# dazzmo/ik

Measured on AMD Instinct MI355X. Metric: IK solves/sec (50-iter DLS) at batch=65536, higher is better.
Workload: dtype f64; 1 GPU; Cassie single-leg chain (cassie_fixed.urdf, 7 support joints of nq=16), one SE(3) LeftFootFront task, 50 fixed DLS iterations, damping 1e-2, step 1.0, reachable targets FK(q*); batch_per_gpu=65536, global_batch=65536, kernel=dls_chain<NJ=7,full,hot>, parallelism=single GPU

## Files before the change

### ik_amd/csrc/device/chain_hot.hpp

```cpp
#pragma once
#if !defined(__HIPCC_RTC__)
#include <cstdint>
#endif

#include "chain_kernel_body.hpp"

namespace ikdev {

constexpr int kStructBits = 21;
constexpr int kStructPerWord = 3;
enum : unsigned { kEntGeneral = 0, kEntZero = 1, kEntOne = 2, kEntMinusOne = 3 };

template <uint64_t C0, uint64_t C1, uint64_t C2>
struct ChainStruct {
    static constexpr uint64_t word(int w) { return w == 0 ? C0 : (w == 1 ? C1 : C2); }
    static constexpr unsigned code(int i) { return static_cast<unsigned>((word(i / kStructPerWord) >> (kStructBits * (i % kStructPerWord))) & 0x1fffffu); }
    static constexpr unsigned ent(int i, int e) { return (code(i) >> (2 * e)) & 3u; }
    static constexpr bool tnz(int i, int k) { return ((code(i) >> (18 + k)) & 1u) != 0; }
    static constexpr int ngen_before(int i, int e) { return e == 0 ? 0 : ngen_before(i, e - 1) + (ent(i, e - 1) == kEntGeneral ? 1 : 0); }
    static constexpr int count(int i) { return ngen_before(i, 9) + (tnz(i, 0) ? 1 : 0) + (tnz(i, 1) ? 1 : 0) + (tnz(i, 2) ? 1 : 0); }
    static constexpr int offset(int i) { return i == 0 ? 0 : offset(i - 1) + count(i - 1); }
    static constexpr int rot_at(int i, int e) { return offset(i) + ngen_before(i, e); }
    static constexpr int trans_at(int i, int k) {
        return offset(i) + ngen_before(i, 9) + (k > 0 && tnz(i, 0) ? 1 : 0) + (k > 1 && tnz(i, 1) ? 1 : 0);
// ... 93 lines not shown
                if (S::tnz(jj, 0)) {                                                                       \
                    const double t0 = t.v[S::trans_at(jj, 0)];                                             \
                    p[0] = dfma(cs[jj], t0, p[0]); p[1] = dfma(-sn[jj], t0, p[1]);                         \
                }                                                                                          \
                if (S::tnz(jj, 1)) {                                                                       \
                    const double t1 = t.v[S::trans_at(jj, 1)];                                             \
                    p[0] = dfma(sn[jj], t1, p[0]); p[1] = dfma(cs[jj], t1, p[1]);                          \
                }                                                                                          \
                if (S::tnz(jj, 2)) p[2] += t.v[S::trans_at(jj, 2)];                                        \
            } else {                                                                                       \
                                       \
                _Pragma("unroll") for (int k = 0; k < 6; ++k) rows[jj][k] = R[k];                          \
                rot_z_left(R, p, sn[jj], cs[jj]);                                                          \
                hot_compose_left<S, jj>(R, p, t);                                                          \
                if (kPinWalk) { IKD_PIN(p[0]); IKD_PIN(p[1]); IKD_PIN(p[2]); IKD_PIN(R[0]); }              \
            }                                                                                              \
        }                                                                                                  \
    }
    IKD_HOT_JOINT(6) IKD_HOT_JOINT(5) IKD_HOT_JOINT(4) IKD_HOT_JOINT(3) IKD_HOT_JOINT(2) IKD_HOT_JOINT(1) IKD_HOT_JOINT(0)
#undef IKD_HOT_JOINT

    if (kRuns.any_folded) { IKD_PIN(p[0]); IKD_PIN(p[1]); }
    double Re[9], pe[3];
#pragma unroll
    for (int i = 0; i < 3; ++i)
#pragma unroll
        for (int j = 0; j < 3; ++j) Re[3 * i + j] = dfma(R[i], oMt[j], dfma(R[3 + i], oMt[3 + j], R[6 + i] * oMt[6 + j]));
    {
        const double dp[3] = {oMt[9] - p[0], oMt[10] - p[1], oMt[11] - p[2]};
        rotT_vec(R, dp, pe);
    }
    LogAndJlog lj;
    double Cm[9];
    log6_and_jlog6_hot<false>(Re, pe, lj, &Cm);
#pragma unroll
    for (int i = 0; i < 6; ++i) e[i] = lj.e[i];

    double Ar0[NJ][3], Ar1[NJ][3];
#pragma unroll
    for (int j = 0; j < NJ; ++j)
        if (kRuns.folded[j] && kRuns.leader[j] == j) {
#pragma unroll
            for (int i = 0; i < 3; ++i) {
                Ar0[j][i] = dfma(lj.A[3 * i], rows[j][0], dfma(lj.A[3 * i + 1], rows[j][1], lj.A[3 * i + 2] * rows[j][2]));
                Ar1[j][i] = dfma(lj.A[3 * i], rows[j][3], dfma(lj.A[3 * i + 1], rows[j][4], lj.A[3 * i + 2] * rows[j][5]));
            }
        }

#pragma unroll
    for (int j = 0; j < NJ; ++j) {
        double beta[3];
#pragma unroll
        for (int i = 0; i < 3; ++i) beta[i] = dfma(lj.A[3 * i], ang[j][0], dfma(lj.A[3 * i + 1], ang[j][1], lj.A[3 * i + 2] * ang[j][2]));
#pragma unroll
        for (int i = 0; i < 3; ++i) {
            const double cb = dfma(Cm[3 * i], beta[0], dfma(Cm[3 * i + 1], beta[1], Cm[3 * i + 2] * beta[2]));
            if (!kRuns.folded[j])
            col[j][i] = dfma(lj.A[3 * i], lin[j][0], dfma(lj.A[3 * i + 1], lin[j][1], dfma(lj.A[3 * i + 2], lin[j][2], cb)));
            else
                col[j][i] = dfma(pt[j][0], Ar1[kRuns.leader[j]][i], dfma(-pt[j][1], Ar0[kRuns.leader[j]][i], cb));
            col[j][3 + i] = beta[i];
        }
    }
}

template <int NJ, class S>
IKD_FN void hot_gram(const double (&col)[NJ][6], double lam2, double (&G)[36]) {
// ... 47 lines not shown
IKD_FN void hot_step(const Tab &t, const LoopParams &prm, const double (&col)[NJ][6], const double (&y)[6], double (&q)[NJ], bool take) {
    constexpr int kLim = S::offset(NJ + 1);
    constexpr typename ChainRuns<S, NJ>::Table kRuns = ChainRuns<S, NJ>::value;
    double ang[NJ];
#pragma unroll
    for (int j = 0; j < NJ; ++j)
        if (kRuns.leader[j] == j) ang[j] = dfma(col[j][3], y[3], dfma(col[j][4], y[4], col[j][5] * y[5]));
#pragma unroll
    for (int j = 0; j < NJ; ++j) {
        double s = ang[kRuns.leader[j]];
#pragma unroll
        for (int a = 0; a < 3; ++a) s = dfma(col[j][a], y[a], s);
        const double qn = dfma(prm.step_length, s, q[j]);
        const double qc = dmin(t.v[kLim + NJ + j], dmax(qn, t.v[kLim + j]));
        q[j] = take ? qc : q[j];
    }
}

template <int NJ, class S, bool NEVERSTOP, class Tab, class AnyFn>
IKD_FN void hot_dls(const Tab &t, const LoopParams &prm, double (&q)[NJ], const double (&oMt)[12], int &iters_out,
                    bool &success_out, AnyFn any_active) {
    constexpr int M = 6;
    bool active = true;
    bool success = false;
    int iters = prm.max_iterations;
#pragma unroll 1
    for (int it = 0; it < prm.max_iterations; ++it) {
        double e[M], col[NJ][M];
        hot_evaluate<NJ, S>(t, q, oMt, e, col);

        double G[M * M];
        hot_gram<NJ, S>(col, prm.lam2, G);
        double y[M];
        chol_solve<M>(G, e, y);

        if (!NEVERSTOP) {
            double e0sq = 0.0;
            if (prm.priority == 0) {
#pragma unroll
                for (int a = 0; a < M; ++a) e0sq = dfma(e[a], e[a], e0sq);
            }
            const bool stop_now = active && (prm.stop_sq_tol >= 0.0) && (e0sq < prm.stop_sq_tol);
            if (stop_now) { success = true; iters = it; }
            active = active && !stop_now;
        }
        hot_step<NJ, S>(t, prm, col, y, q, NEVERSTOP || active);
        if (!NEVERSTOP && !any_active(active)) break;
    }
    iters_out = (NEVERSTOP || success) ? iters : iterations_taken(any_active, prm.max_iterations);
    success_out = success;
}

template <int NJ>
IKD_FN void hot_pass_through_from(const ChainKernelArgs<NJ> &a, const double *q_src, double *q_out, int64_t b, bool stepped) {
    constexpr int kGroup = 16;
    for (int i0 = 0; i0 < a.nq; i0 += kGroup) {
        double v[kGroup], lo[kGroup], hi[kGroup];
        bool out[kGroup];
#pragma unroll
        for (int k = 0; k < kGroup; ++k) {
            const int i = i0 + k < a.nq ? i0 + k : a.nq - 1;
            out[k] = i0 + k < a.nq && !a.q_in_chain[i];
            v[k] = q_src[at(a.layout, a.B, a.nq, i, b)];
            lo[k] = a.lower[i];
            hi[k] = a.upper[i];
        }
#pragma unroll
        for (int k = 0; k < kGroup; ++k) {
            const double c = dmin(hi[k], dmax(v[k], lo[k]));
            if (out[k]) q_out[at(a.layout, a.B, a.nq, i0 + k, b)] = stepped ? c : v[k];
        }
    }
}
template <int NJ>
IKD_FN void hot_pass_through_to(const ChainKernelArgs<NJ> &a, double *q_out, int64_t b, bool stepped) { hot_pass_through_from(a, a.q0, q_out, b, stepped); }
template <int NJ>
IKD_FN void hot_pass_through(const ChainKernelArgs<NJ> &a, int64_t b, bool stepped) { hot_pass_through_to(a, a.q_out, b, stepped); }

#if IKD_HIP_LANG
template <int NJ, class S, class Tab>
__device__ __forceinline__ void hot_refill_body(const ChainKernelArgs<NJ> &a, const Tab &t, unsigned long long *queue, int chunk) {
    chain_refill_loop<NJ>(a, queue, chunk, [&](double (&q)[NJ], const double (&oMt)[12], bool have) {
        constexpr int M = 6;
        double e[M], col[NJ][M];
        hot_evaluate<NJ, S>(t, q, oMt, e, col);
        double G[M * M];
        hot_gram<NJ, S>(col, a.prm.lam2, G);
        double y[M];
        chol_solve<M>(G, e, y);
        double e0sq = 0.0;
        if (a.prm.priority == 0) {
#pragma unroll
            for (int k = 0; k < M; ++k) e0sq = dfma(e[k], e[k], e0sq);
        }
        const bool stop_now = have && (a.prm.stop_sq_tol >= 0.0) && (e0sq < a.prm.stop_sq_tol);
        hot_step<NJ, S>(t, a.prm, col, y, q, !stop_now);
        return stop_now;
    });
}
#endif

template <int NJ, class S, bool NEVERSTOP, class Tab, class AnyFn>
IKD_FN void hot_chain_body(const ChainKernelArgs<NJ> &a, const Tab &t, int64_t gid, AnyFn any_active) {
#if defined(IKGPU_HOT_STAMP) && IKD_ON_DEVICE
    const long long rs = wall_clock64();
#endif
    const bool valid = gid < a.B;
    const int64_t b = valid ? gid : a.B - 1;
    double q[NJ];
#pragma unroll
    for (int j = 0; j < NJ; ++j) q[j] = a.q0[at(a.layout, a.B, a.nq, a.qidx[j], b)];
    double oMt[12];
    load_target(a, b, oMt);
    if (NEVERSTOP && valid) hot_pass_through(a, b, a.prm.max_iterations > 0);
    int iters;
    bool success;
#if defined(IKGPU_HOT_STAMP) && IKD_ON_DEVICE
    const long long c0 = __builtin_readcyclecounter(), r0 = wall_clock64();
#endif
    hot_dls<NJ, S, NEVERSTOP>(t, a.prm, q, oMt, iters, success, any_active);
#if defined(IKGPU_HOT_STAMP) && IKD_ON_DEVICE
    const long long c1 = __builtin_readcyclecounter(), r1 = wall_clock64();
    const int stamp_loop_cycles = static_cast<int>(c1 - c0), stamp_loop_ticks = static_cast<int>(r1 - r0);
    const int stamp_pre_ticks = static_cast<int>(r0 - rs);
    const int stamp_true_iters = iters;
#endif
    if (!NEVERSTOP && a.append_count)
        append_unfinished(a.append_list, a.append_count, valid && !success && iters < a.prm.max_iterations, b);
    if (!valid) return;
#pragma unroll
    for (int j = 0; j < NJ; ++j) a.q_out[at(a.layout, a.B, a.nq, a.qidx[j], b)] = q[j];
    if (!NEVERSTOP) hot_pass_through(a, b, iters > 0);
    if (a.success) a.success[b] = success ? 1 : 0;
#if defined(IKGPU_HOT_STAMP) && IKD_ON_DEVICE
    {
        asm volatile("s_waitcnt vmcnt(0)" ::: "memory");
        const long long re = wall_clock64();
        const int lane = threadIdx.x % 64;
        iters = lane == 0 ? stamp_loop_cycles : lane == 1 ? stamp_loop_ticks : lane == 2 ? stamp_pre_ticks
              : lane == 3 ? static_cast<int>(re - r1) : lane == 4 ? static_cast<int>(rs & 0x7fffffff)
              : lane == 5 ? static_cast<int>(re & 0x7fffffff) : stamp_true_iters;
    }
#endif
    if (a.iters) a.iters[b] = iters;
}

template <int NJ, class S, bool NEVERSTOP, class Tab, class AnyFn>
IKD_FN void hot_track_body(const ChainKernelArgs<NJ> &a, const Tab &t, int T, int64_t gid, AnyFn any_active) {
    const bool valid = gid < a.B;
    const int64_t b = valid ? gid : a.B - 1;
    const int64_t q_slab = static_cast<int64_t>(a.nq) * a.B, t_slab = 12 * a.B;
    double q[NJ];
#pragma unroll
    for (int j = 0; j < NJ; ++j) q[j] = a.q0[at(a.layout, a.B, a.nq, a.qidx[j], b)];
    double next[12], oMt[12];
    if (T > 0) {
        load_target_raw(a, a.targets, b, next);
        compose_target(a, next, oMt);
    }
    if (T > 1) load_target_raw(a, a.targets + t_slab, b, next);
    bool stepped = NEVERSTOP && a.prm.max_iterations > 0;
    for (int k = 0; k < T; ++k) {
        double *q_out = a.q_out + k * q_slab;
        if (NEVERSTOP && valid) hot_pass_through_to(a, q_out, b, stepped);
        int iters;
        bool success;
        hot_dls<NJ, S, NEVERSTOP>(t, a.prm, q, oMt, iters, success, any_active);
        stepped = stepped || iters > 0;
        if (k + 1 < T) compose_target(a, next, oMt);
        if (valid) {
#pragma unroll
            for (int j = 0; j < NJ; ++j) q_out[at(a.layout, a.B, a.nq, a.qidx[j], b)] = q[j];
            if (a.success) a.success[k * a.B + b] = success ? 1 : 0;
            if (a.iters) a.iters[k * a.B + b] = iters;
            if (!NEVERSTOP) hot_pass_through_to(a, q_out, b, stepped);
        }
        if (k + 2 < T) load_target_raw(a, a.targets + (k + 2) * t_slab, b, next);
    }
}

template <int NJ, class S, bool NEVERSTOP, class Tab, class AnyFn>
IKD_FN void hot_multistart_lane(const ChainKernelArgs<NJ> &a, const MultistartArgs &ms, const Tab &t, int64_t b, int k, double (&q)[NJ],
                                bool &success, int &iters, double &err_sq, AnyFn any_active) {
    multistart_load(a, ms, b, k, q);
    double oMt[12];
    load_target(a, b, oMt);
    hot_dls<NJ, S, NEVERSTOP>(t, a.prm, q, oMt, iters, success, any_active);
    double e[6], col[NJ][6];
    hot_evaluate<NJ, S>(t, q, oMt, e, col);
    err_sq = 0.0;
#pragma unroll
    for (int r = 0; r < 6; ++r) err_sq = dfma(e[r], e[r], err_sq);
}

template <int NJ, class S, bool NEVERSTOP, class Tab, class AnyFn, class Exchange>
IKD_FN void hot_multistart_body(const ChainKernelArgs<NJ> &a, const MultistartArgs &ms, const Tab &t, int64_t gid, AnyFn any_active,
                                Exchange exchange) {
    const int64_t prob = gid >> ms.log2K;
    const int k = static_cast<int>(gid & ((int64_t{1} << ms.log2K) - 1));
    const bool valid = prob < a.B;
    const int64_t b = valid ? prob : a.B - 1;
    double q[NJ], err_sq;
    bool success;
    int iters;
    hot_multistart_lane<NJ, S, NEVERSTOP>(a, ms, t, b, k, q, success, iters, err_sq, any_active);
// ... 94 lines not shown
```

### ik_amd/csrc/device/chain_kernel_body.hpp

```cpp
#pragma once
#if !defined(__HIPCC_RTC__)
#include <cstdint>
#endif

#include "chain_solver.hpp"
#include "multistart.hpp"
#include "solutions.hpp"

namespace ikdev {

enum : int { LAYOUT_SOA = 0, LAYOUT_AOS = 1 };

template <int NJ>
struct ChainKernelArgs {
    const ChainDesc<NJ> *desc;
    LoopParams prm;
    double ref_pl[12];
    int qidx[NJ];
    int vidx[NJ];
    int nq, nv, layout;
    int64_t B;
    const double *q0;
    const double *targets;
    double *q_out;
    uint8_t *success;
    int32_t *iters;
    const double *lower, *upper;
    const uint8_t *q_in_chain;
    double *e_out, *J_out, *oMf_out;
    const int32_t *worklist;
    const unsigned long long *count;
    int leave_active, leave_after;
    int32_t *append_list;
    unsigned long long *append_count;
};

IKD_FN void append_unfinished(int32_t *list, unsigned long long *count, bool open, int64_t b) {
#if IKD_ON_DEVICE
    const unsigned long long mask = __ballot(open);
    if (mask == 0ull) return;
    const int lane = static_cast<int>(threadIdx.x) & 63;
    unsigned long long base = 0;
    if (lane == __ffsll(static_cast<long long>(mask)) - 1) base = atomicAdd(count, static_cast<unsigned long long>(__popcll(mask)));
    const int src = __ffsll(static_cast<long long>(mask)) - 1;
    const unsigned lo = __shfl(static_cast<unsigned>(base), src), hi = __shfl(static_cast<unsigned>(base >> 32), src);
    base = (static_cast<unsigned long long>(hi) << 32) | lo;
    if (open) list[base + __popcll(mask & ((1ull << lane) - 1ull))] = static_cast<int32_t>(b);
#else
    if (open) list[(*count)++] = static_cast<int32_t>(b);
#endif
}

IKD_FN int64_t at(int layout, int64_t B, int ncomp, int c, int64_t b) {
    return layout == LAYOUT_SOA ? static_cast<int64_t>(c) * B + b : b * ncomp + c;
}

template <int NJ>
IKD_FN void load_target(const ChainKernelArgs<NJ> &a, int64_t b, double (&oMt)[12]) {
    double t[12];
#pragma unroll
    for (int k = 0; k < 12; ++k) t[k] = a.targets[at(a.layout, a.B, 12, k, b)];
    const double *r = a.ref_pl;
#pragma unroll
    for (int i = 0; i < 3; ++i) {
#pragma unroll
        for (int j = 0; j < 3; ++j)
            oMt[3 * i + j] = dfma(r[3 * i], t[j], dfma(r[3 * i + 1], t[3 + j], r[3 * i + 2] * t[6 + j]));
        oMt[9 + i] = dfma(r[3 * i], t[9], dfma(r[3 * i + 1], t[10], dfma(r[3 * i + 2], t[11], r[9 + i])));
    }
}

template <int NJ, int KT, int SMASK = -1, class Desc, class AnyFn>
IKD_FN void dls_chain_body(const ChainKernelArgs<NJ> &a, const Desc &d, int64_t gid, AnyFn any_active) {
    const bool valid = gid < a.B;
    const int64_t b = valid ? gid : a.B - 1;

    double q[NJ];
#pragma unroll
    for (int j = 0; j < NJ; ++j) q[j] = a.q0[at(a.layout, a.B, a.nq, a.qidx[j], b)];
    double oMt[12];
    load_target(a, b, oMt);

    int iters;
    bool success;
    chain_dls<NJ, KT, SMASK>(d, a.prm, q, oMt, iters, success, any_active);

    if (a.append_count) append_unfinished(a.append_list, a.append_count, valid && !success && iters < a.prm.max_iterations, b);
    if (!valid) return;
#pragma unroll
    for (int j = 0; j < NJ; ++j) a.q_out[at(a.layout, a.B, a.nq, a.qidx[j], b)] = q[j];
    for (int i = 0; i < a.nq; ++i) {
        if (a.q_in_chain[i]) continue;
        const double v = a.q0[at(a.layout, a.B, a.nq, i, b)];
        const double c = dmin(a.upper[i], dmax(v, a.lower[i]));
        a.q_out[at(a.layout, a.B, a.nq, i, b)] = (iters > 0) ? c : v;
    }
    if (a.success) a.success[b] = success ? 1 : 0;
    if (a.iters) a.iters[b] = iters;
}

template <int NJ>
IKD_FN void load_target_raw(const ChainKernelArgs<NJ> &a, const double *targets, int64_t b, double (&t)[12]) {
#pragma unroll
    for (int k = 0; k < 12; ++k) t[k] = targets[at(a.layout, a.B, 12, k, b)];
}
template <int NJ>
IKD_FN void compose_target(const ChainKernelArgs<NJ> &a, const double (&t)[12], double (&oMt)[12]) {
    const double *r = a.ref_pl;
#pragma unroll
    for (int i = 0; i < 3; ++i) {
#pragma unroll
        for (int j = 0; j < 3; ++j)
            oMt[3 * i + j] = dfma(r[3 * i], t[j], dfma(r[3 * i + 1], t[3 + j], r[3 * i + 2] * t[6 + j]));
        oMt[9 + i] = dfma(r[3 * i], t[9], dfma(r[3 * i + 1], t[10], dfma(r[3 * i + 2], t[11], r[9 + i])));
    }
}

template <int NJ, int KT, int SMASK = -1, class Desc, class AnyFn>
IKD_FN void dls_chain_track_body(const ChainKernelArgs<NJ> &a, const Desc &d, int T, int64_t gid, AnyFn any_active) {
    const bool valid = gid < a.B;
    const int64_t b = valid ? gid : a.B - 1;
    const int64_t q_slab = static_cast<int64_t>(a.nq) * a.B, t_slab = 12 * a.B;

    double q[NJ];
#pragma unroll
    for (int j = 0; j < NJ; ++j) q[j] = a.q0[at(a.layout, a.B, a.nq, a.qidx[j], b)];
    double next[12], oMt[12];
    if (T > 0) {
        load_target_raw(a, a.targets, b, next);
        compose_target(a, next, oMt);
    }
    if (T > 1) load_target_raw(a, a.targets + t_slab, b, next);
    bool stepped = false;
    for (int k = 0; k < T; ++k) {
        int iters;
        bool success;
        chain_dls<NJ, KT, SMASK>(d, a.prm, q, oMt, iters, success, any_active);
        stepped = stepped || iters > 0;
        if (k + 1 < T) compose_target(a, next, oMt);
        if (valid) {
            double *q_out = a.q_out + k * q_slab;
#pragma unroll
            for (int j = 0; j < NJ; ++j) q_out[at(a.layout, a.B, a.nq, a.qidx[j], b)] = q[j];
            if (a.success) a.success[k * a.B + b] = success ? 1 : 0;
            if (a.iters) a.iters[k * a.B + b] = iters;
            for (int i = 0; i < a.nq; ++i) {
                if (a.q_in_chain[i]) continue;
                const double v = a.q0[at(a.layout, a.B, a.nq, i, b)];
                const double c = dmin(a.upper[i], dmax(v, a.lower[i]));
                q_out[at(a.layout, a.B, a.nq, i, b)] = stepped ? c : v;
            }
        }
        if (k + 2 < T) load_target_raw(a, a.targets + (k + 2) * t_slab, b, next);
    }
}


template <int NJ>
IKD_FN const double *multistart_source(const ChainKernelArgs<NJ> &a, const MultistartArgs &ms, int k) {
    return (k == 0 || !ms.starts) ? a.q0 : ms.starts + static_cast<int64_t>(k - 1) * a.nq * a.B;
}

template <int NJ>
IKD_FN void multistart_load(const ChainKernelArgs<NJ> &a, const MultistartArgs &ms, int64_t b, int k, double (&q)[NJ]) {
    const double *src = multistart_source(a, ms, k);
    const bool generated = k > 0 && !ms.starts;
#pragma unroll
    for (int j = 0; j < NJ; ++j) {
        const int i = a.qidx[j];
        const double v = src[at(a.layout, a.B, a.nq, i, b)];
        const double r = multistart_draw(ms.seed, b, k, i, a.lower[i], a.upper[i]);
        q[j] = (generated && ms.draw[i]) ? r : v;
    }
}

template <int NJ, int KT, int SMASK = -1, class Desc, class AnyFn>
IKD_FN void dls_chain_multistart_lane(const ChainKernelArgs<NJ> &a, const MultistartArgs &ms, const Desc &d, int64_t b, int k,
                                      double (&q)[NJ], bool &success, int &iters, double &err_sq, AnyFn any_active) {
    constexpr int M = TaskDim<KT>::value;
    multistart_load(a, ms, b, k, q);
    double oMt[12];
    load_target(a, b, oMt);
    chain_dls<NJ, KT, SMASK>(d, a.prm, q, oMt, iters, success, any_active);
    double e[M], col[NJ][M], Rf[9], pf[3];
    chain_evaluate<NJ, KT, SMASK>(d, q, oMt, a.prm.idmask, a.prm.unit_weights != 0, e, col, Rf, pf);
    err_sq = 0.0;
#pragma unroll
    for (int r = 0; r < M; ++r) err_sq = dfma(e[r], e[r], err_sq);
}

template <int NJ, class Pass>
IKD_FN void multistart_store(const ChainKernelArgs<NJ> &a, const MultistartArgs &ms, int64_t b, int k, const double (&q)[NJ], bool success,
                             int iters, double err_sq, Pass pass) {
#pragma unroll
    for (int j = 0; j < NJ; ++j) a.q_out[at(a.layout, a.B, a.nq, a.qidx[j], b)] = q[j];
    pass(multistart_source(a, ms, k), iters > 0);
    if (a.success) a.success[b] = success ? 1 : 0;
    if (a.iters) a.iters[b] = iters;
    if (ms.winner) ms.winner[b] = k;
    if (ms.err_sq) ms.err_sq[b] = err_sq;
}

template <int NJ>
IKD_FN void chain_pass_through_from(const ChainKernelArgs<NJ> &a, const double *src, int64_t b, bool stepped) {
    for (int i = 0; i < a.nq; ++i) {
        if (a.q_in_chain[i]) continue;
        const double v = src[at(a.layout, a.B, a.nq, i, b)];
        const double c = dmin(a.upper[i], dmax(v, a.lower[i]));
        a.q_out[at(a.layout, a.B, a.nq, i, b)] = stepped ? c : v;
    }
}

template <int NJ, int KT, int SMASK = -1, class Desc, class AnyFn, class Exchange>
IKD_FN void dls_chain_multistart_body(const ChainKernelArgs<NJ> &a, const MultistartArgs &ms, const Desc &d, int64_t gid, AnyFn any_active,
                                      Exchange exchange) {
    const int64_t prob = gid >> ms.log2K;
    const int k = static_cast<int>(gid & ((int64_t{1} << ms.log2K) - 1));
    const bool valid = prob < a.B;
    const int64_t b = valid ? prob : a.B - 1;
    double q[NJ], err_sq;
    bool success;
    int iters;
    dls_chain_multistart_lane<NJ, KT, SMASK>(a, ms, d, b, k, q, success, iters, err_sq, any_active);
    const int win = multistart_select(ms.log2K, multistart_key(success, err_sq), k, exchange);
    if (valid && win == k)
        multistart_store(a, ms, b, k, q, success, iters, err_sq, [&](const double *src, bool stepped) { chain_pass_through_from(a, src, b, stepped); });
}


template <int NJ>
IKD_FN void chain_pass_through_into(const ChainKernelArgs<NJ> &a, const double *src, double *q_out, int64_t b, bool stepped) {
    for (int i = 0; i < a.nq; ++i) {
        if (a.q_in_chain[i]) continue;
        const double v = src[at(a.layout, a.B, a.nq, i, b)];
        const double c = dmin(a.upper[i], dmax(v, a.lower[i]));
        q_out[at(a.layout, a.B, a.nq, i, b)] = stepped ? c : v;
    }
}

template <int NJ, int KT, int SMASK = -1, class Desc, class AnyFn>
IKD_FN void dls_chain_solutions_lane(const ChainKernelArgs<NJ> &a, const SolutionsArgs &sa, const Desc &d, int64_t b, int k, double (&q)[NJ],
                                     bool &success, int &iters, AnyFn any_active) {
    multistart_load(a, sa.ms, b, k, q);
    double oMt[12];
    load_target(a, b, oMt);
    chain_dls<NJ, KT, SMASK>(d, a.prm, q, oMt, iters, success, any_active);
}

template <int NJ, class Pass>
IKD_FN void solutions_store(const ChainKernelArgs<NJ> &a, const SolutionsArgs &sa, int64_t b, int k, int slot, const double (&q)[NJ], int iters,
                            Pass pass) {
    double *q_out = a.q_out + static_cast<int64_t>(slot) * a.nq * a.B;
    pass(multistart_source(a, sa.ms, k), q_out, iters > 0);
#pragma unroll
    for (int j = 0; j < NJ; ++j) q_out[at(a.layout, a.B, a.nq, a.qidx[j], b)] = q[j];
    if (sa.which) sa.which[slot * a.B + b] = k;
    if (a.iters) a.iters[slot * a.B + b] = iters;
}

template <int NJ, int KT, int SMASK = -1, class Desc, class AnyFn, class Fetch>
IKD_FN void dls_chain_solutions_body(const ChainKernelArgs<NJ> &a, const SolutionsArgs &sa, const Desc &d, int64_t gid, AnyFn any_active,
                                     Fetch fetch) {
    const int64_t prob = gid >> sa.ms.log2K;
    const int k = static_cast<int>(gid & ((int64_t{1} << sa.ms.log2K) - 1));
    const bool valid = prob < a.B;
    const int64_t b = valid ? prob : a.B - 1;
    double q[NJ];
    bool success;
    int iters;
    dls_chain_solutions_lane<NJ, KT, SMASK>(a, sa, d, b, k, q, success, iters, any_active);
    SolutionsLane s;
    solutions_select<NJ>(s, sa.ms.log2K, k, sa.N, sa.sep, success, q, fetch);
    if (!valid) return;
    if (s.kept)
        solutions_store(a, sa, b, k, s.slot, q, iters,
                        [&](const double *src, double *q_out, bool stepped) { chain_pass_through_into(a, src, q_out, b, stepped); });
    if (k == 0) sa.count[b] = s.cnt;
}

#if IKD_HIP_LANG
template <int NJ, class IterFn>
__device__ __forceinline__ void chain_refill_loop(const ChainKernelArgs<NJ> &a, unsigned long long *queue, int chunk_and_batch, IterFn iterate) {
    const int lane = static_cast<int>(threadIdx.x) & 63;
    const int64_t first_round = static_cast<int64_t>(gridDim.x) * 64;
    const bool listed = a.worklist != nullptr;
    const int64_t nwork = listed ? static_cast<int64_t>(*a.count) : a.B;
    const double *qsrc = listed ? a.q_out : a.q0;
    auto problem = [&](int64_t w) { return listed ? static_cast<int64_t>(a.worklist[w]) : w; };
    const int64_t w0 = static_cast<int64_t>(blockIdx.x) * 64 + lane;
    bool have = w0 < nwork;
    double q[NJ], oMt[12];
    int64_t b = 0;
    int it = 0;
    const int max_it = a.prm.max_iterations;
    const int64_t working = (nwork + 63) / 64 < static_cast<int64_t>(gridDim.x) ? (nwork + 63) / 64 : static_cast<int64_t>(gridDim.x);
    if (static_cast<int64_t>(blockIdx.x) >= working) return;
    b = problem(have ? w0 : 0);
#pragma unroll
    for (int j = 0; j < NJ; ++j) q[j] = qsrc[at(a.layout, a.B, a.nq, a.qidx[j], b)];
    load_target(a, b, oMt);
    if (listed) it = a.iters[b];
    int64_t pool_lo = 0, pool_hi = 0;
    bool exhausted = first_round >= nwork;
    const int batch = chunk_and_batch >> 16, chunk = chunk_and_batch & 0xffff;
    while (__any(have)) {
        const bool stop_now = iterate(q, oMt, have) && have;
        ++it;
        const bool done = have && (stop_now || it >= max_it);
        if (done) {
#pragma unroll
            for (int j = 0; j < NJ; ++j) a.q_out[at(a.layout, a.B, a.nq, a.qidx[j], b)] = q[j];
            if (a.success) a.success[b] = stop_now ? 1 : 0;
            a.iters[b] = stop_now ? it - 1 : max_it;
            have = false;
        }
        const unsigned long long mask = __ballot(!have);
        const int need = __popcll(mask);
        const bool supply = pool_hi > pool_lo || !exhausted;
        if (supply && (need >= batch || need == 64)) {
            const int rank = __popcll(mask & ((1ull << lane) - 1ull));
            const int64_t avail = pool_hi - pool_lo;
            int64_t nb = pool_lo + rank;
            bool got = rank < avail;
            if (avail < need && !exhausted) {
                unsigned long long v = 0;
                if (lane == 0) v = atomicAdd(queue, static_cast<unsigned long long>(chunk));
                const unsigned lo = __builtin_amdgcn_readfirstlane(static_cast<unsigned>(v)), hi = __builtin_amdgcn_readfirstlane(static_cast<unsigned>(v >> 32));
                const int64_t nlo = first_round + static_cast<int64_t>((static_cast<unsigned long long>(hi) << 32) | lo);
                const int64_t nhi = nlo + chunk < nwork ? nlo + chunk : nwork;
                exhausted = nlo + chunk >= nwork;
                if (rank >= avail) { nb = nlo + (rank - avail); got = nb < nhi; }
                pool_lo = nlo + (need - avail);
                pool_hi = nhi > pool_lo ? nhi : pool_lo;
            } else {
                pool_lo += need < avail ? need : avail;
            }
            if (!have && got) {
                have = true;
                b = problem(nb);
#pragma unroll
                for (int j = 0; j < NJ; ++j) q[j] = qsrc[at(a.layout, a.B, a.nq, a.qidx[j], b)];
                load_target(a, b, oMt);
                it = listed ? a.iters[b] : 0;
            }
        }
    }
    if (lane == 0) {
        __threadfence();
        if (atomicAdd(queue + 1, 1ull) == static_cast<unsigned long long>(working) - 1ull) {
            queue[0] = 0ull;
            queue[1] = 0ull;
            queue[2] = 0ull;
            __threadfence();
        }
    }
}

template <int NJ, int KT, int SMASK, class Desc>
__device__ __forceinline__ void dls_chain_refill_body(const ChainKernelArgs<NJ> &a, const Desc &d_in, unsigned long long *queue, int chunk) {
    const Desc *dp = &d_in;
    chain_refill_loop<NJ>(a, queue, chunk, [&](double (&q)[NJ], const double (&oMt)[12], bool) {
        asm volatile("" ::: "memory");
        if constexpr (!std::is_same<Desc, ChainDesc<NJ>>::value) IKD_LAUNDER(dp);
        return chain_iteration<NJ, KT, SMASK>(*dp, a.prm, q, oMt, true);
    });
}

#endif

template <int NJ, int KT>
IKD_FN void eval_chain_body(const ChainKernelArgs<NJ> &a, const ChainDesc<NJ> &d, int64_t b) {
    constexpr int M = TaskDim<KT>::value;
    if (b >= a.B) return;
    double q[NJ];
// ... 42 lines not shown
```

### ik_amd/csrc/device/chain_solver.hpp

```cpp
#pragma once
#if !defined(__HIPCC_RTC__)
#include <type_traits>
#endif

#include "lane_math.hpp"

namespace ikdev {

enum : int { KT_POSITION = 0, KT_ORIENTATION = 1, KT_FULL = 2 };

template <int NJ>
struct ChainDesc {
    double pl[NJ][12];
    double frame_pl[12];
    double lo[NJ], hi[NJ];
    double wgt[6];
};

struct LoopParams {
    int max_iterations;
    double lam2;
    double step_length;
    double stop_sq_tol;
    int priority;
// ... 119 lines not shown
        if (KT == KT_FULL || KT == KT_POSITION) {
#pragma unroll
            for (int i = 0; i < 3; ++i)
                col[j][i] = dfma(AtR[3 * i], vw[0], dfma(AtR[3 * i + 1], vw[1], dfma(AtR[3 * i + 2], vw[2],
                            dfma(BtR[3 * i], zax[j][0], dfma(BtR[3 * i + 1], zax[j][1], BtR[3 * i + 2] * zax[j][2])))));
        }
        if (KT == KT_FULL || KT == KT_ORIENTATION) {
            constexpr int r0 = (KT == KT_FULL) ? 3 : 0;
#pragma unroll
            for (int i = 0; i < 3; ++i)
                col[j][r0 + i] = dfma(AbR[3 * i], zax[j][0], dfma(AbR[3 * i + 1], zax[j][1], AbR[3 * i + 2] * zax[j][2]));
        }
    }
    (void)M;
}

template <int NJ, int KT, int SMASK = -1, class Desc>
IKD_FN bool chain_iteration(const Desc &d, const LoopParams &prm, double (&q)[NJ], const double (&oMt)[12], bool active) {
    constexpr int M = TaskDim<KT>::value;
    double e[M], col[NJ][M], Rf[9], pf[3];
    chain_evaluate<NJ, KT, SMASK>(d, q, oMt, prm.idmask, prm.unit_weights != 0, e, col, Rf, pf);

    double G[M * M];
#pragma unroll
    for (int a = 0; a < M; ++a)
#pragma unroll
        for (int b = 0; b <= a; ++b) {
            double s = (a == b) ? prm.lam2 : 0.0;
#pragma unroll
            for (int j = 0; j < NJ; ++j) s = dfma(col[j][a], col[j][b], s);
            G[a * M + b] = s;
        }
    double y[M];
    chol_solve<M>(G, e, y);

    double e0sq = 0.0;
    if (prm.priority == 0) {
#pragma unroll
        for (int a = 0; a < M; ++a) e0sq = dfma(e[a], e[a], e0sq);
    }
    const bool stop_now = active && (prm.stop_sq_tol >= 0.0) && (e0sq < prm.stop_sq_tol);
    const bool step = active && !stop_now;
#pragma unroll
    for (int j = 0; j < NJ; ++j) {
        double s = 0.0;
#pragma unroll
        for (int a = 0; a < M; ++a) s = dfma(col[j][a], y[a], s);
        const double qn = dfma(prm.step_length, s, q[j]);
        const double qc = dmin(d.hi[j], dmax(qn, d.lo[j]));
        q[j] = step ? qc : q[j];
    }
    return stop_now;
}

struct KeepGoing {
    int leave_active, leave_after, n;
    IKD_FN bool operator()(bool act) {
        ++n;
#if IKD_ON_DEVICE
        const int live = static_cast<int>(__popcll(__ballot(act)));
        return live > (n >= leave_after ? leave_active : 0);
#else
        return act;
#endif
    }
};
template <class F>
// ... 26 lines not shown
```

### ik_amd/csrc/device/lane_math.hpp

```cpp
#pragma once

#if defined(__HIPCC_RTC__)
typedef signed long long int64_t;
typedef unsigned long long uint64_t;
typedef signed int int32_t;
typedef unsigned int uint32_t;
typedef unsigned char uint8_t;
namespace std {
template <class A, class B> struct is_same { static constexpr bool value = false; };
template <class A> struct is_same<A, A> { static constexpr bool value = true; };
template <bool C, class A, class B> struct conditional { typedef A type; };
template <class A, class B> struct conditional<false, A, B> { typedef B type; };
}
#else
#include <cmath>
#include <cstdint>
#endif

#if defined(__HIPCC_RTC__)
#define IKD_FN __host__ __device__ inline __attribute__((always_inline))
#elif defined(__HIPCC__)
#include <hip/hip_runtime.h>
#define IKD_FN __host__ __device__ inline __attribute__((always_inline))
#else
// ... 330 lines not shown
    const double diag = dsel(small, 0.5 * (2.0 - t2 * (1.0 / 6.0)), 0.5 * (theta * st_omc));
#pragma unroll
    for (int i = 0; i < 3; ++i)
#pragma unroll
        for (int j = 0; j < 3; ++j) o.A[3 * i + j] = a3 * u[i] * u[j];
    o.A[0] += diag; o.A[4] += diag; o.A[8] += diag;
    o.A[1] -= 0.5 * u[2]; o.A[2] += 0.5 * u[1];
    o.A[3] += 0.5 * u[2]; o.A[5] -= 0.5 * u[0];
    o.A[6] -= 0.5 * u[1]; o.A[7] += 0.5 * u[0];

    const double inv_t2 = inv_t * inv_t;
    const double bdot = dsel(small, 1.0 / 360.0,
                             dfma(-2.0 * inv_t2, inv_t2, (1.0 + st * inv_t) * inv_t2 * (0.5 * inv_omc)));
    const double up = dot(u, pp);
    const double k1 = bdot * up, k2 = dfma(t2, bdot, 2.0 * beta);
    const double v3[3] = {dfma(k1, u[0], -(k2 * pp[0])), dfma(k1, u[1], -(k2 * pp[1])), dfma(k1, u[2], -(k2 * pp[2]))};
    double C[9];
#pragma unroll
    for (int i = 0; i < 3; ++i)
#pragma unroll
        for (int j = 0; j < 3; ++j) C[3 * i + j] = dfma(v3[i], u[j], beta * u[i] * pp[j]);
    const double ub = up * beta;
    C[0] += ub; C[4] += ub; C[8] += ub;
    C[1] -= 0.5 * pp[2]; C[2] += 0.5 * pp[1];
    C[3] += 0.5 * pp[2]; C[5] -= 0.5 * pp[0];
    C[6] -= 0.5 * pp[1]; C[7] += 0.5 * pp[0];
#pragma unroll
    for (int i = 0; i < 3; ++i)
#pragma unroll
        for (int j = 0; j < 3; ++j)
            o.Bm[3 * i + j] = dfma(C[3 * i], o.A[j], dfma(C[3 * i + 1], o.A[3 + j], C[3 * i + 2] * o.A[6 + j]));
}

template <bool WITH_BM = true>
IKD_FN void log6_and_jlog6_hot(const double (&Re)[9], const double (&pe)[3], LogAndJlog &o, double (*Cout)[9] = nullptr) {
    constexpr double pio2_hi = 1.57079632679489655800e+00, pio2_lo = 6.12323399573676603587e-17;
    constexpr double pS0 = 1.66666666666666657415e-01, pS1 = -3.25565818622400915405e-01,
                     pS2 = 2.01212532134862925881e-01, pS3 = -4.00555345006794114027e-02,
                     pS4 = 7.91534994289814532176e-04, pS5 = 3.47933107596021167570e-05;
    constexpr double qS1 = -2.40339491173441421878e+00, qS2 = 2.02094576023350569471e+00,
                     qS3 = -6.88283971605453293030e-01, qS4 = 7.70381505559019352791e-02;
    const double tr = Re[0] + Re[4] + Re[8];
    double x = dfma(tr, 0.5, -0.5);
    x = dmin(1.0, dmax(-1.0, x));
    const double ax = __builtin_fabs(x);
    const bool mid = ax < 0.5;
    const double z = dfma(-0.5, x, 0.5);
    const double zc = dmax(dfma(0.5, x, 0.5), 0x1p-104);
    const double za = mid ? x * x : dfma(-0.5, ax, 0.5);
    double pp_ = dfma3(za, pS5, pS4);
    pp_ = dfma3(za, pp_, pS3);
    pp_ = dfma3(za, pp_, pS2);
    pp_ = dfma3(za, pp_, pS1);
    pp_ = dfma3(za, pp_, pS0);
    pp_ = pp_ * za;
    double qq = dfma3(za, qS4, qS3);
    qq = dfma3(za, qq, qS2);
    qq = dfma3(za, qq, qS1);
    qq = dfma(za, qq, 1.0);
    const double rr = pp_ * drcp(qq);
    const double sa = dsqrt(za);
    const double tl = dfma(sa, rr, sa);
    const double res_mid = pio2_hi - (x - dfma(-x, rr, pio2_lo));
    const bool pos = x > 0.0;
    const double res_out = dfma(pos ? 2.0 : -2.0, tl, pos ? 0.0 : kPi);
    const double theta = mid ? res_mid : res_out;
    const double h = dsqrt(z * zc);
    const double r = drcp(dmax(theta * h, 1e-300));
    const double inv_t = r * h, inv_h = r * theta;
    const double cot = zc * inv_h;
    const bool small = theta < kTaylorPrec3;
    const double t2 = theta * theta;
    const double inv_t2 = inv_t * inv_t;

    const double fac = dsel(theta > kTaylorPrec3, 0.25 * (theta * inv_h), 0.5);
    double w[3] = {fac * (Re[7] - Re[5]), fac * (Re[2] - Re[6]), fac * (Re[3] - Re[1])};
    const bool near_pi = theta >= kPi - 1e-2;
    if (__builtin_expect(IKD_ANY(near_pi), 0)) {
        const double cphi = -x;
        const double beta_pi = t2 * drcp(2.0 * z);
        const double t0 = (Re[0] + cphi) * beta_pi, t1 = (Re[4] + cphi) * beta_pi, t2v = (Re[8] + cphi) * beta_pi;
        const double a0 = dsel(Re[7] > Re[5], 1.0, -1.0) * dsel(t0 > 0.0, dsqrt(dmax(t0, 0.0)), 0.0);
        const double a1 = dsel(Re[2] > Re[6], 1.0, -1.0) * dsel(t1 > 0.0, dsqrt(dmax(t1, 0.0)), 0.0);
        const double a2 = dsel(Re[3] > Re[1], 1.0, -1.0) * dsel(t2v > 0.0, dsqrt(dmax(t2v, 0.0)), 0.0);
        w[0] = dsel(near_pi, a0, w[0]);
        w[1] = dsel(near_pi, a1, w[1]);
        w[2] = dsel(near_pi, a2, w[2]);
    }

    const double alpha = dsel(small, 1.0 - t2 * (1.0 / 12.0) - t2 * t2 * (1.0 / 720.0), 0.5 * (theta * cot));
    const double beta = dsel(small, 1.0 / 12.0 + t2 * (1.0 / 720.0), dfma(-0.5 * inv_t, cot, inv_t2));
    double wxp[3];
    cross(w, pe, wxp);
    const double bwp = beta * dot(w, pe);
#pragma unroll
    for (int i = 0; i < 3; ++i) {
        o.e[i] = dfma(alpha, pe[i], dfma(-0.5, wxp[i], bwp * w[i]));
        o.e[3 + i] = w[i];
    }

    const double u[3] = {-w[0], -w[1], -w[2]};
    double pp[3];
    rotT_vec(Re, pe, pp);
    pp[0] = -pp[0]; pp[1] = -pp[1]; pp[2] = -pp[2];
    const double a3 = beta;
    const double diag = dsel(small, 0.5 * (2.0 - t2 * (1.0 / 6.0)), 0.5 * (theta * cot));
#pragma unroll
    for (int i = 0; i < 3; ++i)
#pragma unroll
        for (int j = 0; j < 3; ++j) o.A[3 * i + j] = a3 * u[i] * u[j];
    o.A[0] += diag; o.A[4] += diag; o.A[8] += diag;
    o.A[1] -= 0.5 * u[2]; o.A[2] += 0.5 * u[1];
    o.A[3] += 0.5 * u[2]; o.A[5] -= 0.5 * u[0];
    o.A[6] -= 0.5 * u[1]; o.A[7] += 0.5 * u[0];

    const double bdot = dsel(small, 1.0 / 360.0,
                             dfma(-2.0 * inv_t2, inv_t2, dfma(2.0 * h, inv_t, 1.0) * inv_t2 * (0.25 * (cot * inv_h))));
    const double up = dot(u, pp);
    const double k1 = bdot * up, k2 = dfma(t2, bdot, 2.0 * beta);
    const double v3[3] = {dfma(k1, u[0], -(k2 * pp[0])), dfma(k1, u[1], -(k2 * pp[1])), dfma(k1, u[2], -(k2 * pp[2]))};
    double C[9];
#pragma unroll
    for (int i = 0; i < 3; ++i)
#pragma unroll
        for (int j = 0; j < 3; ++j) C[3 * i + j] = dfma(v3[i], u[j], beta * u[i] * pp[j]);
    const double ub = up * beta;
    C[0] += ub; C[4] += ub; C[8] += ub;
    C[1] -= 0.5 * pp[2]; C[2] += 0.5 * pp[1];
    C[3] += 0.5 * pp[2]; C[5] -= 0.5 * pp[0];
    C[6] -= 0.5 * pp[1]; C[7] += 0.5 * pp[0];
    if (WITH_BM) {
#pragma unroll
        for (int i = 0; i < 3; ++i)
#pragma unroll
            for (int j = 0; j < 3; ++j)
                o.Bm[3 * i + j] = dfma(C[3 * i], o.A[j], dfma(C[3 * i + 1], o.A[3 + j], C[3 * i + 2] * o.A[6 + j]));
    } else {
#pragma unroll
        for (int k = 0; k < 9; ++k) (*Cout)[k] = C[k];
    }
}

template <int M>
IKD_FN void chol_solve(double (&G)[M * M], const double (&b)[M], double (&x)[M]) {
    double y[M];
#pragma unroll
    for (int k = 0; k < M; ++k) y[k] = b[k];
#pragma unroll
    for (int k = 0; k < M; ++k) {
        const double inv = drsqrt(G[k * M + k]);
        G[k * M + k] = inv;
        y[k] = y[k] * inv;
#pragma unroll
        for (int i = k + 1; i < M; ++i) G[i * M + k] = G[i * M + k] * inv;
#pragma unroll
        for (int i = k + 1; i < M; ++i) {
#pragma unroll
            for (int j = k + 1; j <= i; ++j) G[i * M + j] = dfma(-G[i * M + k], G[j * M + k], G[i * M + j]);
            y[i] = dfma(-G[i * M + k], y[k], y[i]);
        }
    }
#pragma unroll
    for (int k = M - 1; k >= 0; --k) {
        x[k] = y[k] * G[k * M + k];
#pragma unroll
        for (int m = 0; m < k; ++m) y[m] = dfma(-G[k * M + m], x[k], y[m]);
    }
}

}
```

Before: 660.3 million solves/s.

## Switch to LDLT solve, lean log6 reciprocals, and opaque scalar layout strides

Replaces the Cholesky solve with a square-root-free LDLᵀ solve in the hot and general DLS paths. Adds a LEAN variant of log6/jlog6 that uses rsqrt plus a separate reciprocal instead of sqrt and a combined reciprocal, reuses alpha for the diagonal, and mirrors the symmetric A entries. It also precomputes layout strides once per kernel and pins them to scalar registers with an empty asm, so index math drops the per-access layout branch. Trade-offs: slightly different numerics near theta≈0 and clamps at 2^-200, plus possible register or codegen shifts.

Measured after the change: 687.2 million solves/s (median of 6 runs). 1.04x the previous value.

```diff
diff --git a/ik_amd/csrc/device/chain_hot.hpp b/ik_amd/csrc/device/chain_hot.hpp
--- a/ik_amd/csrc/device/chain_hot.hpp
+++ b/ik_amd/csrc/device/chain_hot.hpp
@@ -149,7 +149,7 @@
     }
     LogAndJlog lj;
     double Cm[9];
-    log6_and_jlog6_hot<false>(Re, pe, lj, &Cm);
+    log6_and_jlog6_hot<false, true>(Re, pe, lj, &Cm);
 #pragma unroll
     for (int i = 0; i < 6; ++i) e[i] = lj.e[i];
 
@@ -263,7 +263,7 @@
         double G[M * M];
         hot_gram<NJ, S>(col, prm.lam2, G);
         double y[M];
-        chol_solve<M>(G, e, y);
+        ldlt_solve<M>(G, e, y);
 
         if (!NEVERSTOP) {
             double e0sq = 0.0;
@@ -284,6 +284,7 @@
 
 template <int NJ>
 IKD_FN void hot_pass_through_from(const ChainKernelArgs<NJ> &a, const double *q_src, double *q_out, int64_t b, bool stepped) {
+    const ChainStrides st = chain_strides(a);
     constexpr int kGroup = 16;
     for (int i0 = 0; i0 < a.nq; i0 += kGroup) {
         double v[kGroup], lo[kGroup], hi[kGroup];
@@ -292,14 +293,18 @@
         for (int k = 0; k < kGroup; ++k) {
             const int i = i0 + k < a.nq ? i0 + k : a.nq - 1;
             out[k] = i0 + k < a.nq && !a.q_in_chain[i];
-            v[k] = q_src[at(a.layout, a.B, a.nq, i, b)];
             lo[k] = a.lower[i];
             hi[k] = a.upper[i];
         }
 #pragma unroll
         for (int k = 0; k < kGroup; ++k) {
+            const int i = i0 + k < a.nq ? i0 + k : a.nq - 1;
+            v[k] = q_src[at(st.elem, st.q_prob, i, b)];
+        }
+#pragma unroll
+        for (int k = 0; k < kGroup; ++k) {
             const double c = dmin(hi[k], dmax(v[k], lo[k]));
-            if (out[k]) q_out[at(a.layout, a.B, a.nq, i0 + k, b)] = stepped ? c : v[k];
+            if (out[k]) q_out[at(st.elem, st.q_prob, i0 + k, b)] = stepped ? c : v[k];
         }
     }
 }
@@ -318,7 +323,7 @@
         double G[M * M];
         hot_gram<NJ, S>(col, a.prm.lam2, G);
         double y[M];
-        chol_solve<M>(G, e, y);
+        ldlt_solve<M>(G, e, y);
         double e0sq = 0.0;
         if (a.prm.priority == 0) {
 #pragma unroll
@@ -333,6 +338,7 @@
 
 template <int NJ, class S, bool NEVERSTOP, class Tab, class AnyFn>
 IKD_FN void hot_chain_body(const ChainKernelArgs<NJ> &a, const Tab &t, int64_t gid, AnyFn any_active) {
+    const ChainStrides st = chain_strides(a);
 #if defined(IKGPU_HOT_STAMP) && IKD_ON_DEVICE
     const long long rs = wall_clock64();
 #endif
@@ -340,7 +346,7 @@
     const int64_t b = valid ? gid : a.B - 1;
     double q[NJ];
 #pragma unroll
-    for (int j = 0; j < NJ; ++j) q[j] = a.q0[at(a.layout, a.B, a.nq, a.qidx[j], b)];
+    for (int j = 0; j < NJ; ++j) q[j] = a.q0[at(st.elem, st.q_prob, a.qidx[j], b)];
     double oMt[12];
     load_target(a, b, oMt);
     if (NEVERSTOP && valid) hot_pass_through(a, b, a.prm.max_iterations > 0);
@@ -360,7 +366,7 @@
         append_unfinished(a.append_list, a.append_count, valid && !success && iters < a.prm.max_iterations, b);
     if (!valid) return;
 #pragma unroll
-    for (int j = 0; j < NJ; ++j) a.q_out[at(a.layout, a.B, a.nq, a.qidx[j], b)] = q[j];
+    for (int j = 0; j < NJ; ++j) a.q_out[at(st.elem, st.q_prob, a.qidx[j], b)] = q[j];
     if (!NEVERSTOP) hot_pass_through(a, b, iters > 0);
     if (a.success) a.success[b] = success ? 1 : 0;
 #if defined(IKGPU_HOT_STAMP) && IKD_ON_DEVICE
@@ -378,12 +384,13 @@
 
 template <int NJ, class S, bool NEVERSTOP, class Tab, class AnyFn>
 IKD_FN void hot_track_body(const ChainKernelArgs<NJ> &a, const Tab &t, int T, int64_t gid, AnyFn any_active) {
+    const ChainStrides st = chain_strides(a);
     const bool valid = gid < a.B;
     const int64_t b = valid ? gid : a.B - 1;
     const int64_t q_slab = static_cast<int64_t>(a.nq) * a.B, t_slab = 12 * a.B;
     double q[NJ];
 #pragma unroll
-    for (int j = 0; j < NJ; ++j) q[j] = a.q0[at(a.layout, a.B, a.nq, a.qidx[j], b)];
+    for (int j = 0; j < NJ; ++j) q[j] = a.q0[at(st.elem, st.q_prob, a.qidx[j], b)];
     double next[12], oMt[12];
     if (T > 0) {
         load_target_raw(a, a.targets, b, next);
@@ -401,7 +408,7 @@
         if (k + 1 < T) compose_target(a, next, oMt);
         if (valid) {
 #pragma unroll
-            for (int j = 0; j < NJ; ++j) q_out[at(a.layout, a.B, a.nq, a.qidx[j], b)] = q[j];
+            for (int j = 0; j < NJ; ++j) q_out[at(st.elem, st.q_prob, a.qidx[j], b)] = q[j];
             if (a.success) a.success[k * a.B + b] = success ? 1 : 0;
             if (a.iters) a.iters[k * a.B + b] = iters;
             if (!NEVERSTOP) hot_pass_through_to(a, q_out, b, stepped);
diff --git a/ik_amd/csrc/device/chain_kernel_body.hpp b/ik_amd/csrc/device/chain_kernel_body.hpp
--- a/ik_amd/csrc/device/chain_kernel_body.hpp
+++ b/ik_amd/csrc/device/chain_kernel_body.hpp
@@ -55,11 +55,31 @@
     return layout == LAYOUT_SOA ? static_cast<int64_t>(c) * B + b : b * ncomp + c;
 }
 
+struct ChainStrides {
+    int64_t elem, q_prob, t_prob;
+};
+#if IKD_ON_DEVICE
+#define IKD_OPAQUE_S(x) asm("" : "+s"(x))
+#else
+#define IKD_OPAQUE_S(x) ((void)0)
+#endif
+template <class Args>
+IKD_FN ChainStrides chain_strides(const Args &a) {
+    const bool soa = a.layout == LAYOUT_SOA;
+    ChainStrides s{soa ? a.B : int64_t{1}, soa ? int64_t{1} : static_cast<int64_t>(a.nq), soa ? int64_t{1} : int64_t{12}};
+    IKD_OPAQUE_S(s.elem);
+    IKD_OPAQUE_S(s.q_prob);
+    IKD_OPAQUE_S(s.t_prob);
+    return s;
+}
+IKD_FN int64_t at(int64_t elem, int64_t prob, int c, int64_t b) { return static_cast<int64_t>(c) * elem + b * prob; }
+
 template <int NJ>
 IKD_FN void load_target(const ChainKernelArgs<NJ> &a, int64_t b, double (&oMt)[12]) {
+    const ChainStrides st = chain_strides(a);
     double t[12];
 #pragma unroll
-    for (int k = 0; k < 12; ++k) t[k] = a.targets[at(a.layout, a.B, 12, k, b)];
+    for (int k = 0; k < 12; ++k) t[k] = a.targets[at(st.elem, st.t_prob, k, b)];
     const double *r = a.ref_pl;
 #pragma unroll
     for (int i = 0; i < 3; ++i) {
@@ -72,12 +92,13 @@
 
 template <int NJ, int KT, int SMASK = -1, class Desc, class AnyFn>
 IKD_FN void dls_chain_body(const ChainKernelArgs<NJ> &a, const Desc &d, int64_t gid, AnyFn any_active) {
+    const ChainStrides st = chain_strides(a);
     const bool valid = gid < a.B;
     const int64_t b = valid ? gid : a.B - 1;
 
     double q[NJ];
 #pragma unroll
-    for (int j = 0; j < NJ; ++j) q[j] = a.q0[at(a.layout, a.B, a.nq, a.qidx[j], b)];
+    for (int j = 0; j < NJ; ++j) q[j] = a.q0[at(st.elem, st.q_prob, a.qidx[j], b)];
     double oMt[12];
     load_target(a, b, oMt);
 
@@ -88,12 +109,12 @@
     if (a.append_count) append_unfinished(a.append_list, a.append_count, valid && !success && iters < a.prm.max_iterations, b);
     if (!valid) return;
 #pragma unroll
-    for (int j = 0; j < NJ; ++j) a.q_out[at(a.layout, a.B, a.nq, a.qidx[j], b)] = q[j];
+    for (int j = 0; j < NJ; ++j) a.q_out[at(st.elem, st.q_prob, a.qidx[j], b)] = q[j];
     for (int i = 0; i < a.nq; ++i) {
         if (a.q_in_chain[i]) continue;
-        const double v = a.q0[at(a.layout, a.B, a.nq, i, b)];
+        const double v = a.q0[at(st.elem, st.q_prob, i, b)];
         const double c = dmin(a.upper[i], dmax(v, a.lower[i]));
-        a.q_out[at(a.layout, a.B, a.nq, i, b)] = (iters > 0) ? c : v;
+        a.q_out[at(st.elem, st.q_prob, i, b)] = (iters > 0) ? c : v;
     }
     if (a.success) a.success[b] = success ? 1 : 0;
     if (a.iters) a.iters[b] = iters;
@@ -101,8 +122,9 @@
 
 template <int NJ>
 IKD_FN void load_target_raw(const ChainKernelArgs<NJ> &a, const double *targets, int64_t b, double (&t)[12]) {
-#pragma unroll
-    for (int k = 0; k < 12; ++k) t[k] = targets[at(a.layout, a.B, 12, k, b)];
+    const ChainStrides st = chain_strides(a);
+#pragma unroll
+    for (int k = 0; k < 12; ++k) t[k] = targets[at(st.elem, st.t_prob, k, b)];
 }
 template <int NJ>
 IKD_FN void compose_target(const ChainKernelArgs<NJ> &a, const double (&t)[12], double (&oMt)[12]) {
@@ -118,13 +140,14 @@
 
 template <int NJ, int KT, int SMASK = -1, class Desc, class AnyFn>
 IKD_FN void dls_chain_track_body(const ChainKernelArgs<NJ> &a, const Desc &d, int T, int64_t gid, AnyFn any_active) {
+    const ChainStrides st = chain_strides(a);
     const bool valid = gid < a.B;
     const int64_t b = valid ? gid : a.B - 1;
     const int64_t q_slab = static_cast<int64_t>(a.nq) * a.B, t_slab = 12 * a.B;
 
     double q[NJ];
 #pragma unroll
-    for (int j = 0; j < NJ; ++j) q[j] = a.q0[at(a.layout, a.B, a.nq, a.qidx[j], b)];
+    for (int j = 0; j < NJ; ++j) q[j] = a.q0[at(st.elem, st.q_prob, a.qidx[j], b)];
     double next[12], oMt[12];
     if (T > 0) {
         load_target_raw(a, a.targets, b, next);
@@ -141,14 +164,14 @@
         if (valid) {
             double *q_out = a.q_out + k * q_slab;
 #pragma unroll
-            for (int j = 0; j < NJ; ++j) q_out[at(a.layout, a.B, a.nq, a.qidx[j], b)] = q[j];
+            for (int j = 0; j < NJ; ++j) q_out[at(st.elem, st.q_prob, a.qidx[j], b)] = q[j];
             if (a.success) a.success[k * a.B + b] = success ? 1 : 0;
             if (a.iters) a.iters[k * a.B + b] = iters;
             for (int i = 0; i < a.nq; ++i) {
                 if (a.q_in_chain[i]) continue;
-                const double v = a.q0[at(a.layout, a.B, a.nq, i, b)];
+                const double v = a.q0[at(st.elem, st.q_prob, i, b)];
                 const double c = dmin(a.upper[i], dmax(v, a.lower[i]));
-                q_out[at(a.layout, a.B, a.nq, i, b)] = stepped ? c : v;
+                q_out[at(st.elem, st.q_prob, i, b)] = stepped ? c : v;
             }
         }
         if (k + 2 < T) load_target_raw(a, a.targets + (k + 2) * t_slab, b, next);
@@ -163,12 +186,13 @@
 
 template <int NJ>
 IKD_FN void multistart_load(const ChainKernelArgs<NJ> &a, const MultistartArgs &ms, int64_t b, int k, double (&q)[NJ]) {
+    const ChainStrides st = chain_strides(a);
     const double *src = multistart_source(a, ms, k);
     const bool generated = k > 0 && !ms.starts;
 #pragma unroll
     for (int j = 0; j < NJ; ++j) {
         const int i = a.qidx[j];
-        const double v = src[at(a.layout, a.B, a.nq, i, b)];
+        const double v = src[at(st.elem, st.q_prob, i, b)];
         const double r = multistart_draw(ms.seed, b, k, i, a.lower[i], a.upper[i]);
         q[j] = (generated && ms.draw[i]) ? r : v;
     }
@@ -192,8 +216,9 @@
 template <int NJ, class Pass>
 IKD_FN void multistart_store(const ChainKernelArgs<NJ> &a, const MultistartArgs &ms, int64_t b, int k, const double (&q)[NJ], bool success,
                              int iters, double err_sq, Pass pass) {
-#pragma unroll
-    for (int j = 0; j < NJ; ++j) a.q_out[at(a.layout, a.B, a.nq, a.qidx[j], b)] = q[j];
+    const ChainStrides st = chain_strides(a);
+#pragma unroll
+    for (int j = 0; j < NJ; ++j) a.q_out[at(st.elem, st.q_prob, a.qidx[j], b)] = q[j];
     pass(multistart_source(a, ms, k), iters > 0);
     if (a.success) a.success[b] = success ? 1 : 0;
     if (a.iters) a.iters[b] = iters;
@@ -203,11 +228,12 @@
 
 template <int NJ>
 IKD_FN void chain_pass_through_from(const ChainKernelArgs<NJ> &a, const double *src, int64_t b, bool stepped) {
+    const ChainStrides st = chain_strides(a);
     for (int i = 0; i < a.nq; ++i) {
         if (a.q_in_chain[i]) continue;
-        const double v = src[at(a.layout, a.B, a.nq, i, b)];
+        const double v = src[at(st.elem, st.q_prob, i, b)];
         const double c = dmin(a.upper[i], dmax(v, a.lower[i]));
-        a.q_out[at(a.layout, a.B, a.nq, i, b)] = stepped ? c : v;
+        a.q_out[at(st.elem, st.q_prob, i, b)] = stepped ? c : v;
     }
 }
 
@@ -230,11 +256,12 @@
 
 template <int NJ>
 IKD_FN void chain_pass_through_into(const ChainKernelArgs<NJ> &a, const double *src, double *q_out, int64_t b, bool stepped) {
+    const ChainStrides st = chain_strides(a);
     for (int i = 0; i < a.nq; ++i) {
         if (a.q_in_chain[i]) continue;
-        const double v = src[at(a.layout, a.B, a.nq, i, b)];
+        const double v = src[at(st.elem, st.q_prob, i, b)];
         const double c = dmin(a.upper[i], dmax(v, a.lower[i]));
-        q_out[at(a.layout, a.B, a.nq, i, b)] = stepped ? c : v;
+        q_out[at(st.elem, st.q_prob, i, b)] = stepped ? c : v;
     }
 }
 
@@ -250,10 +277,11 @@
 template <int NJ, class Pass>
 IKD_FN void solutions_store(const ChainKernelArgs<NJ> &a, const SolutionsArgs &sa, int64_t b, int k, int slot, const double (&q)[NJ], int iters,
                             Pass pass) {
+    const ChainStrides st = chain_strides(a);
     double *q_out = a.q_out + static_cast<int64_t>(slot) * a.nq * a.B;
     pass(multistart_source(a, sa.ms, k), q_out, iters > 0);
 #pragma unroll
-    for (int j = 0; j < NJ; ++j) q_out[at(a.layout, a.B, a.nq, a.qidx[j], b)] = q[j];
+    for (int j = 0; j < NJ; ++j) q_out[at(st.elem, st.q_prob, a.qidx[j], b)] = q[j];
     if (sa.which) sa.which[slot * a.B + b] = k;
     if (a.iters) a.iters[slot * a.B + b] = iters;
 }
@@ -281,6 +309,7 @@
 #if IKD_HIP_LANG
 template <int NJ, class IterFn>
 __device__ __forceinline__ void chain_refill_loop(const ChainKernelArgs<NJ> &a, unsigned long long *queue, int chunk_and_batch, IterFn iterate) {
+    const ChainStrides st = chain_strides(a);
     const int lane = static_cast<int>(threadIdx.x) & 63;
     const int64_t first_round = static_cast<int64_t>(gridDim.x) * 64;
     const bool listed = a.worklist != nullptr;
@@ -297,7 +326,7 @@
     if (static_cast<int64_t>(blockIdx.x) >= working) return;
     b = problem(have ? w0 : 0);
 #pragma unroll
-    for (int j = 0; j < NJ; ++j) q[j] = qsrc[at(a.layout, a.B, a.nq, a.qidx[j], b)];
+    for (int j = 0; j < NJ; ++j) q[j] = qsrc[at(st.elem, st.q_prob, a.qidx[j], b)];
     load_target(a, b, oMt);
     if (listed) it = a.iters[b];
     int64_t pool_lo = 0, pool_hi = 0;
@@ -309,7 +338,7 @@
         const bool done = have && (stop_now || it >= max_it);
         if (done) {
 #pragma unroll
-            for (int j = 0; j < NJ; ++j) a.q_out[at(a.layout, a.B, a.nq, a.qidx[j], b)] = q[j];
+            for (int j = 0; j < NJ; ++j) a.q_out[at(st.elem, st.q_prob, a.qidx[j], b)] = q[j];
             if (a.success) a.success[b] = stop_now ? 1 : 0;
             a.iters[b] = stop_now ? it - 1 : max_it;
             have = false;
@@ -339,7 +368,7 @@
                 have = true;
                 b = problem(nb);
 #pragma unroll
-                for (int j = 0; j < NJ; ++j) q[j] = qsrc[at(a.layout, a.B, a.nq, a.qidx[j], b)];
+                for (int j = 0; j < NJ; ++j) q[j] = qsrc[at(st.elem, st.q_prob, a.qidx[j], b)];
                 load_target(a, b, oMt);
                 it = listed ? a.iters[b] : 0;
             }
diff --git a/ik_amd/csrc/device/chain_solver.hpp b/ik_amd/csrc/device/chain_solver.hpp
--- a/ik_amd/csrc/device/chain_solver.hpp
+++ b/ik_amd/csrc/device/chain_solver.hpp
@@ -175,7 +175,7 @@
             G[a * M + b] = s;
         }
     double y[M];
-    chol_solve<M>(G, e, y);
+    ldlt_solve<M>(G, e, y);
 
     double e0sq = 0.0;
     if (prm.priority == 0) {
diff --git a/ik_amd/csrc/device/lane_math.hpp b/ik_amd/csrc/device/lane_math.hpp
--- a/ik_amd/csrc/device/lane_math.hpp
+++ b/ik_amd/csrc/device/lane_math.hpp
@@ -386,7 +386,7 @@
             o.Bm[3 * i + j] = dfma(C[3 * i], o.A[j], dfma(C[3 * i + 1], o.A[3 + j], C[3 * i + 2] * o.A[6 + j]));
 }
 
-template <bool WITH_BM = true>
+template <bool WITH_BM = true, bool LEAN = false>
 IKD_FN void log6_and_jlog6_hot(const double (&Re)[9], const double (&pe)[3], LogAndJlog &o, double (*Cout)[9] = nullptr) {
     constexpr double pio2_hi = 1.57079632679489655800e+00, pio2_lo = 6.12323399573676603587e-17;
     constexpr double pS0 = 1.66666666666666657415e-01, pS1 = -3.25565818622400915405e-01,
@@ -419,9 +419,18 @@
     const bool pos = x > 0.0;
     const double res_out = dfma(pos ? 2.0 : -2.0, tl, pos ? 0.0 : kPi);
     const double theta = mid ? res_mid : res_out;
-    const double h = dsqrt(z * zc);
-    const double r = drcp(dmax(theta * h, 1e-300));
-    const double inv_t = r * h, inv_h = r * theta;
+    double h, inv_t, inv_h;
+    if (LEAN) {
+        const double zz = z * zc;
+        inv_h = drsqrt(dmax(zz, 0x1p-200));
+        h = zz * inv_h;
+        inv_t = drcp(dmax(theta, 0x1p-200));
+    } else {
+        h = dsqrt(z * zc);
+        const double r = drcp(dmax(theta * h, 1e-300));
+        inv_t = r * h;
+        inv_h = r * theta;
+    }
     const double cot = zc * inv_h;
     const bool small = theta < kTaylorPrec3;
     const double t2 = theta * theta;
@@ -458,11 +467,11 @@
     rotT_vec(Re, pe, pp);
     pp[0] = -pp[0]; pp[1] = -pp[1]; pp[2] = -pp[2];
     const double a3 = beta;
-    const double diag = dsel(small, 0.5 * (2.0 - t2 * (1.0 / 6.0)), 0.5 * (theta * cot));
+    const double diag = LEAN ? alpha : dsel(small, 0.5 * (2.0 - t2 * (1.0 / 6.0)), 0.5 * (theta * cot));
 #pragma unroll
     for (int i = 0; i < 3; ++i)
 #pragma unroll
-        for (int j = 0; j < 3; ++j) o.A[3 * i + j] = a3 * u[i] * u[j];
+        for (int j = 0; j < 3; ++j) o.A[3 * i + j] = (LEAN && j < i) ? o.A[3 * j + i] : a3 * u[i] * u[j];
     o.A[0] += diag; o.A[4] += diag; o.A[8] += diag;
     o.A[1] -= 0.5 * u[2]; o.A[2] += 0.5 * u[1];
     o.A[3] += 0.5 * u[2]; o.A[5] -= 0.5 * u[0];
@@ -522,4 +531,33 @@
     }
 }
 
-}
+template <int M>
+IKD_FN void ldlt_solve(double (&G)[M * M], const double (&b)[M], double (&x)[M]) {
+    double y[M];
+#pragma unroll
+    for (int k = 0; k < M; ++k) y[k] = b[k];
+#pragma unroll
+    for (int k = 0; k < M; ++k) {
+        const double inv = drcp(G[k * M + k]);
+        G[k * M + k] = inv;
+#pragma unroll
+        for (int i = k + 1; i < M; ++i) {
+            const double l = G[i * M + k] * inv;
+#pragma unroll
+            for (int j = k + 1; j <= i; ++j) G[i * M + j] = dfma(-l, G[j * M + k], G[i * M + j]);
+            y[i] = dfma(-l, y[k], y[i]);
+        }
+#pragma unroll
+        for (int i = k + 1; i < M; ++i) G[i * M + k] = G[i * M + k] * inv;
+    }
+#pragma unroll
+    for (int k = 0; k < M; ++k) y[k] = y[k] * G[k * M + k];
+#pragma unroll
+    for (int k = M - 1; k >= 0; --k) {
+        x[k] = y[k];
+#pragma unroll
+        for (int m = 0; m < k; ++m) y[m] = dfma(-G[k * M + m], x[k], y[m]);
+    }
+}
+
+}
```
